# ygjwd12345/UCD

Measured on AMD Instinct MI355X. Metric: images/sec (whole node) per UCD train step, VOC 15-5 step-1, 513^2 bs=24, higher is better.
Workload: dtype bf16

## Files before the change

### include/ucd_hip.h

```cpp
#ifndef UCD_HIP_H
#define UCD_HIP_H

#include <stddef.h>
#include <stdint.h>

#ifdef __cplusplus
extern "C" {
#endif

#define UCD_VERSION 100

typedef void* ucd_stream_t;
typedef void* ucd_comm_t;

enum ucd_dtype { UCD_F32 = 0, UCD_BF16 = 1 };
enum ucd_act { UCD_ACT_IDENTITY = 0, UCD_ACT_LEAKY_RELU = 1, UCD_ACT_ELU = 2  };
#define UCD_ACT_MASK 0xff
#define UCD_NORM_ABS_GAMMA 0x100
enum ucd_pixcon_precision { UCD_PIXCON_F32 = 0, UCD_PIXCON_F16 = 1, UCD_PIXCON_F16_SPLIT = 2 };
enum ucd_error {
  UCD_OK = 0,
  UCD_EINVAL = -1,
  UCD_EALIGN = -2,
  UCD_EWORKSPACE = -3,
// ... 324 lines not shown
int ucd_abn_reduce_partials(const float* partial, int tiles, int C, float* sums, float* sums_copy, const float* weight,
                            int flags, ucd_stream_t stream);

size_t ucd_conv1x1_wgrad_workspace_bytes(int M, int N, int K);
int ucd_conv1x1_wgrad(const void* dy, int ld_dy, const void* a, int lda, int M, int N, int K,
                      const float* in_mean, const float* in_scale, const float* in_shift, int in_act, float in_slope,
                      void* dw, void* workspace, size_t workspace_bytes, ucd_stream_t stream);

int ucd_abn_sync_finalize(const float* gathered, int world, int M, int C, const float* weight, float* running_mean,
                          float* running_var, float momentum, float eps, float* buf, int flags, ucd_stream_t stream);

int ucd_stem_conv7x7(const float* x, long long sb, long long sc, long long sh, long long sw, int B, int H, int W, const void* w,
                     void* z, ucd_stream_t stream);

int ucd_stem_conv_pool(const float* x, long long sb, long long sc, long long sh, long long sw, int B, int H, int W, const void* w,
                       const float* mean, const float* scale, const float* beta, int act, float slope, void* out, ucd_stream_t stream);
int ucd_stem_pooled_size(int n);
size_t ucd_stem_pool_workspace_bytes(int C);
int ucd_stem_apply_pool(const void* z, int B, int H, int W, int C, const float* mean, const float* scale, const float* beta, int act,
                        float slope, void* out, uint8_t* idx, ucd_stream_t stream);
int ucd_stem_pool_backward(const void* z, const void* dpool, const uint8_t* idx, int B, int H, int W, int C, const float* mean,
                           const float* invstd, const float* scale, const float* beta, const float* weight, float* sums, float count,
                           int act, float slope, void* dz, void* workspace, size_t workspace_bytes, int phase, ucd_stream_t stream);

size_t ucd_conv_wgrad_workspace_bytes(int M, int N, int K, int taps);
int ucd_conv_wgrad_ex(const void* dz, int ld_dz, const void* x, int ld_x, int M, int N, int K, int taps, int H, int W, int dilation,
                      int stride, void* dw, float* dw32, int accumulate32, void* workspace, size_t workspace_bytes, int flags,
                      ucd_stream_t stream);
int ucd_conv_wgrad_defer(int mode);
int ucd_conv_wgrad_mode(void);
int ucd_conv_wgrad_flush(ucd_stream_t stream);
int ucd_conv_wgrad_drop(ucd_stream_t stream);
int ucd_conv_wgrad_drop_all(void);

enum ucd_wgrad_form {
  UCD_WGRAD_TILE = 0,
  UCD_WGRAD_STRIDED = 1,
  UCD_WGRAD_ROW3 = 2
};
#define UCD_WGRAD_FORM_NAMES {"tile", "strided", "row3"}
typedef struct ucd_conv_wgrad_plan_t {
  int form;
  int tile_n, tile_k, tiles_n, tiles_k;
  int chunks, rows_per_chunk, ksplit;
  int x_tile_rows;
  int grid, threads, lds_bytes;
// ... 60 lines not shown
```

### ucd_amd/abn.py

```python
from __future__ import annotations

import os

from . import switches as _switches

import torch
import torch.distributed as dist
import torch.nn as nn
from torch.optim.optimizer import register_optimizer_step_post_hook

from . import hip
from .comm import direct_comm


def _act_code(name):
    try:
        return hip.ACT_CODES[name]
    except KeyError:
        raise RuntimeError(f"activation {name!r} is not supported by the HIP ABN (leaky_relu, elu, identity)") from None


_param_epoch = [0]


def _after_optimizer_step(optimizer, args, kwargs):
# ... 252 lines not shown

    @staticmethod
    def forward(ctx, x):
        x, M, Cc, HW, ld = hip.rows_view(x)
        B = x.shape[0]
        out = torch.empty(B, Cc, dtype=torch.float32, device=x.device)
        hip.plane_sum(x, ld, B, HW, Cc, 1.0 / HW, out)
        ctx.shape, ctx.dtype = x.shape, x.dtype
        return out.to(x.dtype).view(B, Cc, 1, 1)

    @staticmethod
    def backward(ctx, g):
        B, Cc, H, W = ctx.shape
        return (g.to(ctx.dtype) / (H * W)).expand(B, Cc, H, W)


def global_avg_pool(x):
    return _PlaneMean.apply(x)


class _StemABNPoolFunction(torch.autograd.Function):

    @staticmethod
    def forward(ctx, z, weight, bias, running_mean, running_var, training, momentum, eps, act, slope, group, eval_consts):
        B, Cc, H, W = z.shape
        M, HW = B * H * W, H * W
        zr, _, _, _, ld = hip.rows_view(z)
        dev = z.device
        world = _group_size(group) if training else 1
        sync = training and group is not False and (world > 1 or (_FORCE_SYNC and dist.is_initialized()))
        if training:
            buf = torch.empty(((8 + 2 * world) if sync else 6) * Cc, dtype=torch.float32, device=dev)
            if sync:
                pack = buf[6 * Cc:8 * Cc]
                hip.abn_sync_stats(zr, ld, M, Cc, None, HW, buf[:2 * Cc], buf[2 * Cc:3 * Cc], pack)
                comm = direct_comm(group)
                if comm is not None:
                    gathered = buf[8 * Cc:]
                    hip._check(hip.load().ucd_comm_all_gather(comm.handle, hip.ptr(pack), hip.ptr(gathered), 2 * Cc, hip.stream()),
                               "ucd_comm_all_gather")
                else:
                    gathered = _all_gather_stats(pack, world, group)
                hip.abn_sync_finalize(gathered, world, M, Cc, weight, running_mean, running_var, momentum, eps, buf, act)
            else:
                hip.abn_stats_finalize(zr, ld, M, Cc, None, HW, buf[:2 * Cc], buf[2 * Cc:3 * Cc], weight, running_mean, running_var,
                                       momentum, eps, buf[3 * Cc:4 * Cc], buf[4 * Cc:5 * Cc], buf[5 * Cc:6 * Cc], act)
            mean, invstd, scale = buf[3 * Cc:4 * Cc], buf[4 * Cc:5 * Cc], buf[5 * Cc:6 * Cc]
        else:
            mean, invstd, scale = running_mean, eval_consts[0], eval_consts[1]
        need_bwd = any(ctx.needs_input_grad[:3])
        out, idx = hip.stem_apply_pool(z, mean, scale, bias, act, slope, need_bwd)
        if need_bwd:
            ctx.save_for_backward(z, idx, weight, bias, mean, invstd, scale)
            ctx.cfg = (training, act, slope, group, world, sync, float(M * world))
        return out

    @staticmethod
    def backward(ctx, dp):
        z, idx, weight, bias, mean, invstd, scale = ctx.saved_tensors
        training, act, slope, group, world, sync, count = ctx.cfg
        if not training:
            raise RuntimeError("ucd_amd.abn: the fused stem has no frozen-statistics backward (fix_bn keeps the separate layers)")
        Cc = z.shape[1]
        if dp.dtype != z.dtype:
            dp = dp.to(z.dtype)
        if not dp.is_contiguous(memory_format=torch.channels_last):
            dp = dp.contiguous(memory_format=torch.channels_last)
        sums = torch.empty(2 * Cc, dtype=torch.float32, device=z.device)
        dz = torch.empty_like(z) if ctx.needs_input_grad[0] else None
        if not sync:
            hip.stem_pool_backward(z, dp, idx, mean, invstd, scale, bias, weight, sums, count, act, slope, dz, 3 if dz is not None else 1)
            dbias, dweight = sums[:Cc], sums[Cc:]
        else:
            hip.stem_pool_backward(z, dp, idx, mean, invstd, scale, bias, weight, sums, count, act, slope, None, 1)
            local = sums.clone()
            dbias, dweight = local[:Cc], local[Cc:]
            comm = direct_comm(group)
            if comm is not None:
                hip._check(hip.load().ucd_comm_all_reduce_sum(comm.handle, hip.ptr(sums), 2 * Cc, hip.stream()), "ucd_comm_all_reduce_sum")
            else:
                _all_reduce_sums(sums, group)
            if dz is not None:
                hip.stem_pool_backward(z, dp, idx, mean, invstd, scale, bias, weight, sums, count, act, slope, dz, 2)
        return (dz, dweight if weight is not None else None, dbias if bias is not None else None) + (None,) * 9


def stem_norm_pool(bn, z):
    import os
    if _switches.get("UCD_STEM_FOLD", "1") == "0" or not getattr(bn, "ucd_fused_abn", False):
        return None
    Cc = z.shape[1] if z.dim() == 4 else 0
    if not (z.is_cuda and z.dim() == 4 and z.dtype == torch.bfloat16 and z.is_contiguous(memory_format=torch.channels_last)
            and z.shape[2] > 2 and z.shape[3] > 2 and Cc % 8 == 0 and 2048 % max(Cc, 1) == 0
            and bn.activation in ("leaky_relu", "identity")):
        return None
    needs_grad = torch.is_grad_enabled() and (z.requires_grad or (bn.weight is not None and bn.weight.requires_grad))
    if needs_grad and not bn.training:
        return None
    act = _act_code(bn.activation) | (hip.NORM_ABS_GAMMA if bn._abs_gamma else 0)
    if bn.training:
        bn.__dict__.pop("_eval_cache", None)
    return _StemABNPoolFunction.apply(z, bn.weight, bn.bias, bn.running_mean, bn.running_var, bn.training, bn.momentum, bn.eps, act,
                                      bn.activation_param, bn._group(), None if bn.training else bn._eval_constants())


class ABN(nn.Module):

    ucd_fused_abn = True
    _inplace_contract = False
    _sync = False
    _abs_gamma = False

    def __init__(self, num_features, eps=1e-5, momentum=0.1, affine=True, activation="leaky_relu",
                 activation_param=0.01, group=None):
        super().__init__()
        self.num_features, self.eps, self.momentum, self.affine = num_features, eps, momentum, affine
        self.activation, self.activation_param = activation, activation_param
        self.group = group
        if affine:
            self.weight = nn.Parameter(torch.ones(num_features))
            self.bias = nn.Parameter(torch.zeros(num_features))
        else:
            self.register_parameter("weight", None)
            self.register_parameter("bias", None)
        self.register_buffer("running_mean", torch.zeros(num_features))
        self.register_buffer("running_var", torch.ones(num_features))
# ... 92 lines not shown
```

### ucd_amd/backbone.py

```python
from __future__ import annotations

import sys
from collections import OrderedDict
from functools import partial

import torch
import torch.nn as nn

from . import switches as _switches
from .blocks import Conv2d, ResidualBlock, try_index

_STAGE_DILATION = {16: (1, 1, 1, 2), 8: (1, 1, 2, 4)}


class GlobalAvgPool2d(nn.Module):

    def forward(self, inputs):
        return inputs.flatten(2).mean(dim=2)


class ResNet(nn.Module):
    def __init__(self, structure, bottleneck, norm_act=nn.BatchNorm2d, classes=0,
                 output_stride=16, keep_outputs=False):
        super().__init__()
# ... 34 lines not shown
                from .abn import stem_norm_pool
                y = _stem_eval_fused(m.conv1, m.bn1, x)
                if y is not None:
                    return y
                z = _stem_conv(m.conv1, x)
                y = stem_norm_pool(m.bn1, z)
                return y if y is not None else pool(m.bn1(z))
        return m(x)

    def forward(self, x, taps=False):
        outs = [self._stem(x)]
        for name in ("mod2", "mod3", "mod4", "mod5"):
            y = getattr(self, name)(outs[-1])
            if taps and name != "mod5" and hasattr(y, "_ucd_blink"):
                del y._ucd_blink
            outs.append(y)
        if taps:
            return outs[4], tuple(outs[1:5])
        if hasattr(self, "classifier"):
            outs.append(self.classifier(outs[-1]))
        return outs if self.keep_outputs else outs[-1]


class _StemConvFunction(torch.autograd.Function):

    @staticmethod
    def forward(ctx, x, w):
        from . import hip
        ctx.save_for_backward(x, w)
        return hip.stem_conv7x7(x, w)

    @staticmethod
    def backward(ctx, dz):
        x, w = ctx.saved_tensors
        dw = None
        if ctx.needs_input_grad[1]:
            xb = x.to(torch.bfloat16).contiguous(memory_format=torch.channels_last)
            dw = torch.ops.aten.convolution_backward(dz.contiguous(memory_format=torch.channels_last), xb, w, None, [2, 2], [3, 3],
                                                     [1, 1], False, [0, 0], 1, [False, True, False])[1]
        return None, dw


def _stem_conv(conv, x):
    w = conv.working_weight() if hasattr(conv, "working_weight") else None
    if w is None and x.is_cuda and torch.is_autocast_enabled() and torch.get_autocast_dtype("cuda") == torch.bfloat16:
        w = conv.weight.to(torch.bfloat16)
    if (w is None or not x.is_cuda or x.dim() != 4 or x.dtype != torch.float32 or x.requires_grad or conv.bias is not None
            or tuple(conv.weight.shape) != (64, 3, 7, 7) or conv.stride != (2, 2) or conv.padding != (3, 3)
            or conv.dilation != (1, 1) or w.dtype != torch.bfloat16 or not w.is_contiguous(memory_format=torch.channels_last)
            or _switches.get("UCD_OWN_STEM", "1") == "0"):
        return conv(x)
    if torch.is_grad_enabled() and w.requires_grad:
        return _StemConvFunction.apply(x, w)
    from . import hip
    return hip.stem_conv7x7(x, w)


def _stem_eval_fused(conv, bn, x):
    from . import abn as _abn
    if (torch.is_grad_enabled() or bn.training or _switches.get("UCD_STEM_EVAL_FUSED", "1") == "0" or _switches.get("UCD_OWN_STEM", "1") == "0"
            or _switches.get("UCD_STEM_FOLD", "1") == "0" or not getattr(bn, "ucd_fused_abn", False)
            or bn.activation not in ("leaky_relu", "identity")):
        return None
# ... 21 lines not shown
```

### ucd_amd/csrc/stem.hip

```cpp
#include "common.h"

namespace ucd {
namespace {

typedef __hip_bfloat16 bf16;
constexpr int kThreads = 256;
constexpr int kRedBlocks = 1024;
constexpr int kApplyRows = 4;

__device__ __forceinline__ float leaky(float z, float slope) { return z > 0.f ? z : z * slope; }
__device__ __forceinline__ float bf16_round(float v) { return __bfloat162float(__float2bfloat16(v)); }

struct StemArgs {
  const bf16* z; int B, H, W, C, PH, PW;
  const float *mean, *scale, *beta, *invstd, *weight, *sums;
  float slope, inv_count;
  int abs_gamma, cg_shift;
};

__global__ __launch_bounds__(kThreads) void stem_apply_pool_kernel(StemArgs p, bf16* __restrict__ out, uint8_t* __restrict__ idx) {
  const int cgs = p.cg_shift, CG = 1 << cgs;
  const int t = blockIdx.x * kThreads + threadIdx.x;
  const int cg = t & (CG - 1), pw = t >> cgs, ph = blockIdx.y, b = blockIdx.z;
  if (pw >= p.PW) return;
// ... 419 lines not shown
    }
    __syncthreads();
    for (int i = tid; i < kFPH * kFPW * 8; i += kThreads) {
      const int cg = i & 7, pp = i >> 3, pr = pp / kFPW, pc = pp - pr * kFPW;
      const int ph = (oy0 + 1) / 2 + pr, pw = (ox0 + 1) / 2 + pc;
      if (ph >= q.PH || pw >= q.PW) continue;
      float best[8];
#pragma unroll
      for (int e = 0; e < 8; ++e) best[e] = -INFINITY;
#pragma unroll
      for (int kh = 0; kh < 3; ++kh)
#pragma unroll
        for (int kw = 0; kw < 3; ++kw) {
          Vec<bf16> v;
          v.raw = *reinterpret_cast<const uint4*>(Tl + ((2 * pr + kh) * kSTW + 2 * pc + kw) * kFTP + cg * 8);
#pragma unroll
          for (int e = 0; e < 8; ++e) best[e] = fmaxf(best[e], v.get(e));
        }
      Vec<bf16> o;
#pragma unroll
      for (int e = 0; e < 8; ++e) o.set(e, best[e]);
      o.store(q.out + (((size_t)b * q.PH + ph) * q.PW + pw) * 64 + cg * 8);
    }
  }
}

bool stem_args_ok(const void* z, int B, int H, int W, int C) {
  return z && B > 0 && B < 65536 && H > 1 && H < 65536 && W > 1 && C >= 8 && (C & (C - 1)) == 0 && C <= 2048 && aligned16(z);
}

}
}

using namespace ucd;

extern "C" {

int ucd_stem_pooled_size(int n) { return (n + 2 - 3) / 2 + 1; }

size_t ucd_stem_pool_workspace_bytes(int C) { return (size_t)kRedBlocks * 2 * C * sizeof(float); }

int ucd_stem_apply_pool(const void* z, int B, int H, int W, int C, const float* mean, const float* scale, const float* beta, int act,
                        float slope, void* out, uint8_t* idx, ucd_stream_t stream) {
  static const char* fn = "ucd_stem_apply_pool";
  UCD_REQUIRE(stem_args_ok(z, B, H, W, C) && mean && scale && out && aligned16(out) && (!idx || (reinterpret_cast<uintptr_t>(idx) & 7) == 0),
              UCD_EINVAL, "%s: dense channels-last bf16 maps with a power-of-two channel count in 8..2048 expected", fn);
// ... 54 lines not shown
  StemArgs p{};
  p.z = (const bf16*)z; p.B = B; p.H = H; p.W = W; p.C = C; p.PH = ucd_stem_pooled_size(H); p.PW = ucd_stem_pooled_size(W);
  p.mean = mean; p.scale = scale; p.beta = beta; p.invstd = invstd; p.weight = weight; p.sums = sums;
  p.slope = a == UCD_ACT_IDENTITY ? 1.f : slope; p.abs_gamma = (act & UCD_NORM_ABS_GAMMA) != 0;
  p.cg_shift = __builtin_ctz(C / 8);
  hipStream_t s = (hipStream_t)stream;
  if (phase & 1) {
    UCD_REQUIRE(workspace && workspace_bytes >= ucd_stem_pool_workspace_bytes(C), UCD_EWORKSPACE, "%s: workspace too small", fn);
    stem_pool_bwd_reduce_kernel<<<kRedBlocks, kThreads, kThreads * 16 * sizeof(float), s>>>(p, (const bf16*)dpool, idx, (float*)workspace);
    int rc = check_launch(fn);
    if (rc) return rc;
    stem_sum_partials_kernel<<<2 * C, kThreads, 0, s>>>((const float*)workspace, kRedBlocks, C, p.abs_gamma ? weight : nullptr, sums);
    rc = check_launch(fn);
    if (rc) return rc;
  }
  if (phase & 2) {
    p.inv_count = 1.f / count;
    stem_pool_bwd_apply_kernel<<<dim3(ceil_div(((W + 1) / 2) * (C / 8), kThreads), ceil_div(H, kApplyRows), B), kThreads, 0, s>>>(p, (const bf16*)dpool, idx, (bf16*)dz);
    return check_launch(fn);
  }
  return 0;
}

}
```

### ucd_amd/hip.py

```python
from __future__ import annotations

import ctypes as C
import os

import torch

_HERE = os.path.dirname(os.path.abspath(__file__))
LIB_PATH = os.path.join(_HERE, "libucd_hip.so")

F32, BF16 = 0, 1
ACT_IDENTITY, ACT_LEAKY_RELU, ACT_ELU = 0, 1, 2
ACT_CODES = {"identity": ACT_IDENTITY, "leaky_relu": ACT_LEAKY_RELU, "elu": ACT_ELU}
ACT_MASK = 0xFF
NORM_ABS_GAMMA = 0x100
PIX_TILE = 128
PIXCON_LD = 256
PIXCON_F32, PIXCON_F16, PIXCON_F16_SPLIT = 0, 1, 2
KD_UNBIASED, KD_PLAIN = 0, 1
EINVAL, EALIGN, EWORKSPACE = -1, -2, -3
EUNSUPPORTED = -4
SEG_FORMS = {1: "pk<16,8>", 2: "pk<20,4>", 3: "pk<12,12>", 4: "reg<24,16>", 5: "reg<24,24>", 6: "wide/fixed", 7: "wide/f32"}
PIXCON_PATHS = {1: "f32", 2: "f32/wide", 3: "f16/planned", 4: "f16/split"}
CONV_FORMS = ("single", "2x64", "lw/128", "lw/256", "lw/64")
WGRAD_FORMS = ("tile", "strided", "row3")
PIXCON_PRECISION = {"f32": PIXCON_F32, "fp32": PIXCON_F32, "f16": PIXCON_F16, "fp16": PIXCON_F16,
                    "f16_split": PIXCON_F16_SPLIT}


class PixconMeta(C.Structure):
    _fields_ = [("A", C.c_int32), ("Co", C.c_int32), ("min_new", C.c_int32), ("n_new", C.c_int32),
# ... 8 lines not shown

class Conv1x1Desc(C.Structure):
    _fields_ = [("a", C.c_void_p), ("lda", C.c_int), ("w", C.c_void_p), ("ldw", C.c_int), ("y", C.c_void_p), ("ldy", C.c_int),
                ("M", C.c_int), ("N", C.c_int), ("K", C.c_int),
                ("in_mean", C.c_void_p), ("in_scale", C.c_void_p), ("in_shift", C.c_void_p), ("in_act", C.c_int),
                ("in_slope", C.c_float), ("out_mode", C.c_int),
                ("out_mean", C.c_void_p), ("out_scale", C.c_void_p), ("out_shift", C.c_void_p), ("out_invstd", C.c_void_p),
                ("residual", C.c_void_p), ("ldr", C.c_int), ("out_act", C.c_int), ("out_slope", C.c_float),
                ("partial", C.c_void_p), ("accumulate", C.c_int),
                ("taps", C.c_int), ("H", C.c_int), ("W", C.c_int), ("dilation", C.c_int),
                ("side2", C.c_void_p), ("ld2", C.c_int), ("stride", C.c_int),
                ("stat_acc", C.c_void_p), ("stat_shift", C.c_void_p), ("stat_acc2", C.c_void_p), ("stat_rep", C.c_int)]


class Conv1x1Plan(C.Structure):
    _fields_ = [(n, C.c_int) for n in ("form", "tile_rows", "tile_cols", "tiles_m", "tiles_n", "grid", "threads", "lds_bytes",
                                       "param_off")]


class Conv_WgradPlan(C.Structure):
    _fields_ = [(n, C.c_int) for n in ("form", "tile_n", "tile_k", "tiles_n", "tiles_k", "chunks", "rows_per_chunk", "ksplit",
                                       "x_tile_rows", "grid", "threads", "lds_bytes", "sum_lanes", "sum_blocks")] + \
               [("workspace_bytes", C.c_size_t)]


_p, _i, _f, _z = C.c_void_p, C.c_int, C.c_float, C.c_size_t
SIGNATURES = {
    "ucd_version": (_i, []),
    "ucd_last_error": (C.c_char_p, []),
    "ucd_abn_workspace_bytes": (_z, [_i, _i]),
    "ucd_abn_stats": (_i, [_p, _i, _i, _i, _i, _p, _i, _p, _p, _p, _z, _p]),
    "ucd_abn_stats_finalize": (_i, [_p, _i, _i, _i, _i, _p, _i, _p, _p, _p, _p, _p, _f, _f, _p, _p, _p, _i, _p, _z, _p]),
    "ucd_abn_finalize": (_i, [_p, _p, _f, _i, _p, _p, _p, _f, _f, _p, _p, _p, _i, _p]),
    "ucd_abn_eval_params": (_i, [_p, _p, _f, _i, _p, _p, _i, _p]),
    "ucd_abn_apply": (_i, [_p, _i, _p, _i, _p, _i, _i, _i, _i, _p, _i, _p, _p, _p, _i, _f, _p]),
    "ucd_conv1x1_stat_replicas": (_i, [_i]),
    "ucd_fill_zero": (_i, [_p, _z, _p]),
    "ucd_abn_apply_stats": (_i, [_p, _i, _p, _i, _p, _i, _i, _i, _p, _i, _p, _f, _p, _p, _p, _p, _f, _f, _p, _p, _p, _i, _f, _p]),
    "ucd_abn_bwd_apply_raw": (_i, [_p, _i, _p, _i, _p, _i, _p, _i, _p, _i, _i, _i, _p, _p, _p, _p, _p, _p, _p, _i, _p, _f, _i, _f, _p]),
    "ucd_abn_bwd_reduce": (_i, [_p, _i, _p, _i, _p, _i, _i, _i, _i, _p, _i, _p, _p, _p, _p, _p, _i, _f, _p, _p, _z, _p]),
    "ucd_label_path": (_i, [_p, _p, _i, _i, _p, _p, _p, _p]),
    "ucd_image_path": (_i, [_p, _p, _i, _i, _i, _i, _f, _f, _f, _f, _f, _f, _p, _p, _p, _p]),
    "ucd_batch_path": (_i, [_p, _p, _p, _i, _i, _p, _f, _f, _f, _f, _f, _f, _p, _p, _p]),
    "ucd_val_image_path": (_i, [_p, _p, _i, _i, _i, _i, _i, _i, _f, _f, _f, _f, _f, _f, _p, _p, _p, _p]),
    "ucd_val_label_path": (_i, [_p, _p, _i, _i, _i, _p, _p, _p, _p]),
    "ucd_gemm_load": (_i, [C.c_char_p]),
# ... 35 lines not shown
    "ucd_attn_mse_workspace_bytes": (_z, [_i, _i]),
    "ucd_attn_mse": (_i, [_p, _i, _p, _i, _i, _i, _i, _i, _f, _p, _p, _i, _p, _z, _p]),
    "ucd_pod_plan": (_i, [_i, _i, _i, _p, _i, _i, _i, _p, _p, _p]),
    "ucd_pod_forward": (_i, [_p, _i, _p, _i, _i, _i, _i, _i, _i, _f, _p, _i, _f, _p, _p, _p, _z, _p]),
    "ucd_pod_backward": (_i, [_p, _i, _i, _i, _i, _i, _i, _f, _p, _i, _p, _p, _p, _i, _p]),
    "ucd_conv1x1_row_tiles": (_i, [_i]),
    "ucd_conv1x1_stats_partial_bytes": (_z, [_i, _i]),
    "ucd_conv1x1": (_i, [C.POINTER(Conv1x1Desc), _p]),
    "ucd_conv1x1_plan": (_i, [C.POINTER(Conv1x1Desc), C.POINTER(Conv1x1Plan)]),
    "ucd_conv1x1_stats_finalize": (_i, [_p, _i, _i, _p, _p, _p, _f, _f, _p, _p, _i, _p]),
    "ucd_conv3_tap_plan": (_i, [_i, _i, _i, _i, _i, _p, _p, _p]),
    "ucd_conv3_tap_classes": (_i, [_i]),
    "ucd_conv3_tap_plans_resident": (_i, []),
    "ucd_conv3_tap_stats": (_i, [_p, _p, _p]),
    "ucd_abn_reduce_partials": (_i, [_p, _i, _i, _p, _p, _p, _i, _p]),
    "ucd_conv1x1_wgrad_workspace_bytes": (_z, [_i, _i, _i]),
    "ucd_conv1x1_wgrad": (_i, [_p, _i, _p, _i, _i, _i, _i, _p, _p, _p, _i, _f, _p, _p, _z, _p]),
    "ucd_abn_sync_finalize": (_i, [_p, _i, _i, _i, _p, _p, _p, _f, _f, _p, _i, _p]),
    "ucd_stem_pooled_size": (_i, [_i]),
    "ucd_stem_pool_workspace_bytes": (_z, [_i]),
    "ucd_stem_apply_pool": (_i, [_p, _i, _i, _i, _i, _p, _p, _p, _i, _f, _p, _p, _p]),
    "ucd_stem_pool_backward": (_i, [_p, _p, _p, _i, _i, _i, _i, _p, _p, _p, _p, _p, _p, _f, _i, _f, _p, _p, _z, _i, _p]),
    "ucd_conv_wgrad_workspace_bytes": (_z, [_i, _i, _i, _i]),
    "ucd_stem_conv7x7": (_i, [_p, C.c_longlong, C.c_longlong, C.c_longlong, C.c_longlong, _i, _i, _i, _p, _p, _p]),
    "ucd_stem_conv_pool": (_i, [_p, C.c_longlong, C.c_longlong, C.c_longlong, C.c_longlong, _i, _i, _i, _p, _p, _p, _p, _i, _f, _p, _p]),
    "ucd_conv_wgrad_ex": (_i, [_p, _i, _p, _i, _i, _i, _i, _i, _i, _i, _i, _i, _p, _p, _i, _p, _z, _i, _p]),
    "ucd_conv_wgrad_defer": (_i, [_i]),
    "ucd_conv_wgrad_mode": (_i, []),
    "ucd_conv_wgrad_flush": (_i, [_p]),
    "ucd_conv_wgrad_drop": (_i, [_p]),
    "ucd_conv_wgrad_drop_all": (_i, []),
    "ucd_conv_wgrad_plan": (_i, [_i, _i, _i, _i, _i, _i, _i, _i, C.POINTER(Conv_WgradPlan)]),
    "ucd_transpose_bf16": (_i, [_p, _i, _i, _p, _p]),
    "ucd_conv_f32": (_i, [_p, _i, _p, _i, _p, _i, _i, _i, _i, _i, _i, _i, _i, _i, _p]),
    "ucd_conv_f32_wgrad_workspace_bytes": (_z, [_i, _i, _i, _i]),
    "ucd_conv_f32_wgrad": (_i, [_p, _i, _p, _i, _i, _i, _i, _i, _i, _i, _i, _p, _p, _z, _p]),
    "ucd_flip_weights_batched": (_i, [_p, _p, _p, _i, _p, _p]),
    "ucd_flip_weights_batched64": (_i, [_p, _p, _p, _i, _p, _p]),
    "ucd_sgd_chunk": (_i, []),
    "ucd_sgd_step": (_i, [_p, _p, _i, _p, _p]),
    "ucd_sgd_hyper_store": (_i, [_p, _p, _p]),
    "ucd_sgd_step_dev": (_i, [_p, _p, _i, _p, _p]),
    "ucd_reg_chunk": (_i, []),
    "ucd_reg_hyper_store": (_i, [_p, _p, _p]),
    "ucd_reg_step": (_i, [_p, _p, _i, _i, _p, _p, _p, _p]),
    "ucd_pixcon_prep_workspace_bytes": (_z, [_i, _i]),
# ... 582 lines not shown
    lib = load()
    B, Cc, H, W = z.shape
    PH, PW = lib.ucd_stem_pooled_size(H), lib.ucd_stem_pooled_size(W)
    out = torch.empty((B, Cc, PH, PW), dtype=z.dtype, device=z.device, memory_format=torch.channels_last)
    idx = torch.empty((B, PH, PW, Cc), dtype=torch.uint8, device=z.device) if want_idx else None
    with _timed("ucd_stem_apply_pool", (z.numel() + out.numel()) * 2 + (idx.numel() if idx is not None else 0)):
        _check(lib.ucd_stem_apply_pool(ptr(z), B, H, W, Cc, ptr(mean), ptr(scale), ptr(beta), act, float(slope), ptr(out), ptr(idx),
                                       stream()), "ucd_stem_apply_pool")
    return out, idx


def stem_pool_backward(z, dpool, idx, mean, invstd, scale, beta, weight, sums, count, act, slope, dz, phase):
    lib = load()
    B, Cc, H, W = z.shape
    nbytes = lib.ucd_stem_pool_workspace_bytes(Cc)
    ws = workspace(nbytes, z.device)
    work = (z.numel() * (2 if phase & 1 else 0) + (2 * z.numel() * 2 if phase & 2 else 0) + dpool.numel() * 3 * (1 + (phase == 3)))
    with _timed("ucd_stem_pool_backward", work):
        _check(lib.ucd_stem_pool_backward(ptr(z), ptr(dpool), ptr(idx), B, H, W, Cc, ptr(mean), ptr(invstd), ptr(scale), ptr(beta),
                                          ptr(weight), ptr(sums), float(count), act, float(slope), ptr(dz), ptr(ws), nbytes,
                                          int(phase), stream()), "ucd_stem_pool_backward")


def wgrad_defer(mode):
    return int(load().ucd_conv_wgrad_defer(int(mode) & 3))


def _wgrad_side_release(stream=None):
    from . import abn as _abn
    node = _abn._abn_node()
    if node is not None:
        node.wgrad_side_release(stream)


def wgrad_flush():
    s = stream()
    _check(load().ucd_conv_wgrad_flush(s), "ucd_conv_wgrad_flush")
    _wgrad_side_release(s)


def wgrad_drop():
    s = stream()
    rc = load().ucd_conv_wgrad_drop(s)
    if rc == 0:
        _wgrad_side_release(s)
    return rc
# ... 140 lines not shown
```

### ucd_amd/switches.py

```python
from __future__ import annotations

import os

DEFAULTS = {
    "UCD_FUSED_CONV1X1": "1",
    "UCD_BWD_LINK": "1",
    "UCD_BLOCK_LINK": "1",
    "UCD_PROJ_ALIAS": "1",
    "UCD_DGRAD_VIA_FWD": "1",
    "UCD_OWN_STRIDED": "1",
    "UCD_OWN_WGRAD": "1",
    "UCD_F32_OWN_CONV": "0",
    "UCD_OWN_HEADS": "1",
    "UCD_OWN_STEM": "1",
    "UCD_WGRAD3": "1",
    "UCD_CONV_PIPE": "auto",
    "UCD_CONV_BN64_TILES": "128",
    "UCD_CONV_LW64_TILES": "128",
    "UCD_WGRAD_DEFER": "1",
    "UCD_WGRAD_STREAM": "1",
    "UCD_CONV3_TAP_CLASSES": "1",
    "UCD_STAT_ATOMIC": "1",
    "UCD_SEG_PK": "1",
    "UCD_SEG_KD_EX": "1",
    "UCD_FUSED_LDE": "1",
    "UCD_FUSED_POD": "1",
    "UCD_VAL_DEVICE": "1",
    "UCD_STEM_EVAL_FUSED": "1",
    "UCD_STEM_FOLD": "1",
    "UCD_ABN_NODE": "1",
    "UCD_SGD": "hip",
    "UCD_STEP_GRAPH": "auto",
    "UCD_TEACHER_OVERLAP": "1",
    "UCD_DIRECT_RCCL": "1",
    "UCD_IPC_SYNC": "auto",
    "UCD_IPC_TIMEOUT_MS": "60000",
    "UCD_DDP_LATE_COPY": "1",
    "UCD_DDP_DIRECT": "auto",
    "UCD_FORCE_COLLECTIVES": "0",
}

_cache: dict = {}


def get(name: str, default: str | None = None) -> str:
    v = _cache.get(name)
    if v is None:
        if default is None:
            default = DEFAULTS.get(name, "")
        v = _cache[name] = os.environ.get(name, default)
    return v

# ... 18 lines not shown
```

Measured before the change: 845.6.

## Fuse stem pool/ABN backward with 7x7 conv weight gradient in one MFMA kernel

```diff
diff --git a/include/ucd_hip.h b/include/ucd_hip.h
--- a/include/ucd_hip.h
+++ b/include/ucd_hip.h
@@ -370,6 +370,17 @@
 int ucd_stem_pool_backward(const void* z, const void* dpool, const uint8_t* idx, int B, int H, int W, int C, const float* mean,
                            const float* invstd, const float* scale, const float* beta, const float* weight, float* sums, float count,
                            int act, float slope, void* dz, void* workspace, size_t workspace_bytes, int phase, ucd_stream_t stream);
+
+typedef struct ucd_stem_wgrad_plan_t {
+  int OH, OW, tiles_y, tiles_x, tiles, min_tiles, workgroups, lds_bytes, supported, qualifies;
+  size_t workspace_bytes;
+} ucd_stem_wgrad_plan_t;
+int ucd_stem_wgrad_plan(int B, int H, int W, int workgroups, ucd_stem_wgrad_plan_t* plan);
+int ucd_stem_pool_backward_wgrad(const void* z, const void* dpool, const uint8_t* idx, int B, int OH, int OW, const float* mean,
+                                 const float* invstd, const float* scale, const float* beta, const float* weight, float* sums,
+                                 float count, int act, float slope, const void* dz, const float* x, long long sb, long long sc,
+                                 long long sh, long long sw, int H, int W, void* dw, void* workspace, size_t workspace_bytes,
+                                 int phase, int workgroups, ucd_stream_t stream);
 
 size_t ucd_conv_wgrad_workspace_bytes(int M, int N, int K, int taps);
 int ucd_conv_wgrad_ex(const void* dz, int ld_dz, const void* x, int ld_x, int M, int N, int K, int taps, int H, int W, int dilation,
diff --git a/ucd_amd/abn.py b/ucd_amd/abn.py
--- a/ucd_amd/abn.py
+++ b/ucd_amd/abn.py
@@ -1,6 +1,7 @@
 from __future__ import annotations
 
 import os
+import weakref
 
 from . import switches as _switches
 
@@ -299,7 +300,8 @@
 class _StemABNPoolFunction(torch.autograd.Function):
 
     @staticmethod
-    def forward(ctx, z, weight, bias, running_mean, running_var, training, momentum, eps, act, slope, group, eval_consts):
+    def forward(ctx, z, weight, bias, running_mean, running_var, training, momentum, eps, act, slope, group, eval_consts,
+                link, zref):
         B, Cc, H, W = z.shape
         M, HW = B * H * W, H * W
         zr, _, _, _, ld = hip.rows_view(z)
@@ -330,6 +332,7 @@
         if need_bwd:
             ctx.save_for_backward(z, idx, weight, bias, mean, invstd, scale)
             ctx.cfg = (training, act, slope, group, world, sync, float(M * world))
+            ctx.link, ctx.zref = link, zref
         return out
 
     @staticmethod
@@ -344,6 +347,26 @@
         if not dp.is_contiguous(memory_format=torch.channels_last):
             dp = dp.contiguous(memory_format=torch.channels_last)
         sums = torch.empty(2 * Cc, dtype=torch.float32, device=z.device)
+        link = ctx.link
+        if link is not None and ctx.needs_input_grad[0]:
+            zt = ctx.zref() if ctx.zref is not None else None
+            if zt is None or not (zt.retains_grad or zt._backward_hooks):
+                args = dict(z=z, dpool=dp, idx=idx, mean=mean, invstd=invstd, scale=scale, beta=bias, weight=weight, sums=sums,
+                            count=count, act=act, slope=slope)
+                if not sync:
+                    link.dw = hip.stem_pool_backward_wgrad(link.x, phase=3, **args)
+                    dbias, dweight = sums[:Cc], sums[Cc:]
+                else:
+                    hip.stem_pool_backward(z, dp, idx, mean, invstd, scale, bias, weight, sums, count, act, slope, None, 1)
+                    local = sums.clone()
+                    dbias, dweight = local[:Cc], local[Cc:]
+                    comm = direct_comm(group)
+                    if comm is not None:
+                        hip._check(hip.load().ucd_comm_all_reduce_sum(comm.handle, hip.ptr(sums), 2 * Cc, hip.stream()), "ucd_comm_all_reduce_sum")
+                    else:
+                        _all_reduce_sums(sums, group)
+                    link.dw = hip.stem_pool_backward_wgrad(link.x, phase=2, **args)
+                return (None, dweight if weight is not None else None, dbias if bias is not None else None) + (None,) * 11
         dz = torch.empty_like(z) if ctx.needs_input_grad[0] else None
         if not sync:
             hip.stem_pool_backward(z, dp, idx, mean, invstd, scale, bias, weight, sums, count, act, slope, dz, 3 if dz is not None else 1)
@@ -359,7 +382,7 @@
                 _all_reduce_sums(sums, group)
             if dz is not None:
                 hip.stem_pool_backward(z, dp, idx, mean, invstd, scale, bias, weight, sums, count, act, slope, dz, 2)
-        return (dz, dweight if weight is not None else None, dbias if bias is not None else None) + (None,) * 9
+        return (dz, dweight if weight is not None else None, dbias if bias is not None else None) + (None,) * 11
 
 
 def stem_norm_pool(bn, z):
@@ -377,8 +400,10 @@
     act = _act_code(bn.activation) | (hip.NORM_ABS_GAMMA if bn._abs_gamma else 0)
     if bn.training:
         bn.__dict__.pop("_eval_cache", None)
+    link = z.__dict__.pop("_ucd_stem_link", None)
     return _StemABNPoolFunction.apply(z, bn.weight, bn.bias, bn.running_mean, bn.running_var, bn.training, bn.momentum, bn.eps, act,
-                                      bn.activation_param, bn._group(), None if bn.training else bn._eval_constants())
+                                      bn.activation_param, bn._group(), None if bn.training else bn._eval_constants(),
+                                      link, weakref.ref(z) if link is not None else None)
 
 
 class ABN(nn.Module):
diff --git a/ucd_amd/backbone.py b/ucd_amd/backbone.py
--- a/ucd_amd/backbone.py
+++ b/ucd_amd/backbone.py
@@ -80,23 +80,43 @@
         return outs if self.keep_outputs else outs[-1]
 
 
+class StemLink:
+    __slots__ = ("x", "dw")
+
+    def __init__(self, x):
+        self.x, self.dw = x, None
+
+
 class _StemConvFunction(torch.autograd.Function):
 
     @staticmethod
     def forward(ctx, x, w):
         from . import hip
         ctx.save_for_backward(x, w)
-        return hip.stem_conv7x7(x, w)
+        z = hip.stem_conv7x7(x, w)
+        ctx.link = None
+        if ctx.needs_input_grad[1] and hip.stem_wgrad_mode(x):
+            ctx.link = z._ucd_stem_link = StemLink(x)
+            ctx.set_materialize_grads(False)
+        return z
 
     @staticmethod
     def backward(ctx, dz):
         x, w = ctx.saved_tensors
         dw = None
+        if dz is None:
+            if ctx.link is not None:
+                dw, ctx.link.dw = ctx.link.dw, None
+            return None, dw
         if ctx.needs_input_grad[1]:
-            xb = x.to(torch.bfloat16).contiguous(memory_format=torch.channels_last)
-            dw = torch.ops.aten.convolution_backward(dz.contiguous(memory_format=torch.channels_last), xb, w, None, [2, 2], [3, 3],
-                                                     [1, 1], False, [0, 0], 1, [False, True, False])[1]
+            dw = _stem_wgrad_library(x, w, dz)
         return None, dw
+
+
+def _stem_wgrad_library(x, w, dz):
+    xb = x.to(torch.bfloat16).contiguous(memory_format=torch.channels_last)
+    return torch.ops.aten.convolution_backward(dz.contiguous(memory_format=torch.channels_last), xb, w, None, [2, 2], [3, 3],
+                                               [1, 1], False, [0, 0], 1, [False, True, False])[1]
 
 
 def _stem_conv(conv, x):
diff --git a/ucd_amd/csrc/stem.hip b/ucd_amd/csrc/stem.hip
--- a/ucd_amd/csrc/stem.hip
+++ b/ucd_amd/csrc/stem.hip
@@ -465,6 +465,195 @@
       for (int e = 0; e < 8; ++e) o.set(e, best[e]);
       o.store(q.out + (((size_t)b * q.PH + ph) * q.PW + pw) * 64 + cg * 8);
     }
+  }
+}
+
+constexpr int kGP = 264;
+constexpr int kWgradSlab = 64 * kSK;
+constexpr int kWgradMaxWgs = 512;
+constexpr int kWgradMinTiles = 256;
+constexpr int kWgradLds = (kSIR * kSIP + 64 * kGP) * 2 + 7 * 64 * 4;
+constexpr int kSumOuts = 16, kSumParts = kThreads / kSumOuts;
+
+struct StemWgradArgs {
+  StemArgs s;
+  const bf16* dpool; const uint8_t* idx;
+  const bf16* dz;
+  const float* x; long long sb, sc, sh, sw;
+  float* slabs;
+  int IH, IW, tiles_y, tiles_x, ntiles;
+};
+
+template <bool FUSED>
+__global__ __launch_bounds__(kThreads, 2) void stem_pool_bwd_wgrad_kernel(StemWgradArgs q) {
+  typedef float f32x16 __attribute__((ext_vector_type(16)));
+  typedef __bf16 bf16x8 __attribute__((ext_vector_type(8)));
+  __shared__ __attribute__((aligned(16))) unsigned short In[kSIR * kSIP];
+  __shared__ __attribute__((aligned(16))) unsigned short Gt[64 * kGP];
+  const StemArgs& p = q.s;
+  const int tid = threadIdx.x, lane = tid & 63, wave = tid >> 6;
+  const int col = lane & 31, h = lane >> 5;
+  const int cg = tid & 7, cp = (tid >> 3) & 15, qr = tid >> 7;
+  __shared__ float Pc[7 * 64];
+  if (FUSED && tid < 64) {
+    const int ch = tid;
+    const float sc = p.scale[ch], is = p.invstd[ch];
+    float k1 = p.sums[p.C + ch] * p.inv_count, gw;
+    if (p.abs_gamma) {
+      if (p.weight && p.weight[ch] < 0.f) k1 = -k1;
+      gw = sc;
+    } else {
+      gw = (p.weight ? p.weight[ch] : 1.f) * is;
+    }
+    Pc[ch] = p.mean[ch]; Pc[64 + ch] = sc; Pc[128 + ch] = p.beta ? p.beta[ch] : 0.f; Pc[192 + ch] = is;
+    Pc[256 + ch] = p.sums[ch] * p.inv_count; Pc[320 + ch] = k1; Pc[384 + ch] = gw;
+  }
+  const int nb = wave & 1, kb0 = (wave >> 1) * 3;
+  int pbase[3];
+#pragma unroll
+  for (int j = 0; j < 3; ++j) {
+    const int kc = (kb0 + j) * 32 + col, ky = kc / 24 > 6 ? 6 : kc / 24;
+    pbase[j] = ky * kSIP + (kc % 24) + 48 * h;
+  }
+  f32x16 acc[3];
+#pragma unroll
+  for (int j = 0; j < 3; ++j)
+#pragma unroll
+    for (int r = 0; r < 16; ++r) acc[j][r] = 0.f;
+  const int fe = tid < kSIP ? tid : kSIP - 1, fpx = fe / 3, fc = fe - fpx * 3;
+  float pre[kSIR];
+  unsigned premask = 0;
+  auto fetch = [&](int tile) {
+    unsigned okm = 0;
+    const int b = tile / (q.tiles_y * q.tiles_x), rem = tile - b * q.tiles_y * q.tiles_x;
+    const int oy0 = (rem / q.tiles_x) * kSTH, ox0 = (rem % q.tiles_x) * kSTW;
+    const int ix = 2 * ox0 - 3 + fpx;
+    const bool colok = fpx < 2 * kSTW + 5 && (unsigned)ix < (unsigned)q.IW;
+    const float* src = q.x + b * q.sb + fc * q.sc + (colok ? ix : 0) * q.sw;
+#pragma unroll
+    for (int r = 0; r < kSIR; ++r) {
+      const int iy = 2 * oy0 - 3 + r;
+      const bool ok = colok && (unsigned)iy < (unsigned)q.IH;
+      pre[r] = src[(ok ? iy : 0) * q.sh];
+      okm |= ok ? (1u << r) : 0u;
+    }
+    premask = okm;
+  };
+  if ((int)blockIdx.x < q.ntiles) fetch(blockIdx.x);
+  for (int tile = blockIdx.x; tile < q.ntiles; tile += gridDim.x) {
+    const int b = tile / (q.tiles_y * q.tiles_x), rem = tile - b * q.tiles_y * q.tiles_x;
+    const int oy0 = (rem / q.tiles_x) * kSTH, ox0 = (rem % q.tiles_x) * kSTW;
+    const int y0 = oy0 + kApplyRows * qr, i = ox0 / 2 + cp, x0 = 2 * i, phb = y0 / 2;
+    Vec<bf16> g[3][2], v[kApplyRows][2];
+    uint2 w[3][2];
+    bool gv[3][2];
+    if (FUSED) {
+#pragma unroll
+      for (int a = 0; a < 3; ++a)
+#pragma unroll
+        for (int c = 0; c < 2; ++c) {
+          gv[a][c] = phb + a < p.PH && i + c < p.PW;
+          const size_t off = (((size_t)b * p.PH + min(phb + a, p.PH - 1)) * p.PW + min(i + c, p.PW - 1)) * p.C + cg * 8;
+          w[a][c] = *reinterpret_cast<const uint2*>(q.idx + off);
+          g[a][c].load(q.dpool + off);
+        }
+    }
+    const bf16* vsrc = FUSED ? p.z : q.dz;
+#pragma unroll
+    for (int r = 0; r < kApplyRows; ++r)
+#pragma unroll
+      for (int cx = 0; cx < 2; ++cx)
+        v[r][cx].load(vsrc + (((size_t)b * p.H + min(y0 + r, p.H - 1)) * p.W + min(x0 + cx, p.W - 1)) * p.C + cg * 8);
+    __syncthreads();
+    if (tid < kSIP) {
+#pragma unroll
+      for (int r = 0; r < kSIR; ++r) {
+        const bf16 t = __float2bfloat16((premask >> r) & 1u ? pre[r] : 0.f);
+        In[r * kSIP + tid] = *reinterpret_cast<const unsigned short*>(&t);
+      }
+    }
+#pragma unroll
+    for (int e = 0; e < 8; ++e) {
+      const int ch = cg * 8 + e;
+      float mu = 0.f, sc = 0.f, sh = 0.f, is = 0.f, k0 = 0.f, k1 = 0.f, gw = 0.f;
+      if (FUSED) { mu = Pc[ch]; sc = Pc[64 + ch]; sh = Pc[128 + ch]; is = Pc[192 + ch]; k0 = Pc[256 + ch]; k1 = Pc[320 + ch]; gw = Pc[384 + ch]; }
+      unsigned* dst = reinterpret_cast<unsigned*>(&Gt[ch * kGP + kApplyRows * qr * kSTW + 2 * cp]);
+#pragma unroll
+      for (int r = 0; r < kApplyRows; ++r) {
+        unsigned bits[2];
+#pragma unroll
+        for (int cx = 0; cx < 2; ++cx) {
+          const bool inside = y0 + r < p.H && x0 + cx < p.W;
+          if (FUSED) {
+            float dy = 0.f;
+#pragma unroll
+            for (int ya = 0; ya < 2; ++ya) {
+              if (ya == 1 && !(r & 1)) continue;
+              const int a = (r >> 1) + ya, kh = (r & 1) ? (ya ? 0 : 2) : 1;
+#pragma unroll
+              for (int xa = 0; xa < 2; ++xa) {
+                if (xa == 1 && !cx) continue;
+                const int kw = cx ? (xa ? 0 : 2) : 1;
+                const unsigned pos = gv[a][xa] ? (unsigned)(kh * 3 + kw) : 0xffu;
+                const unsigned id = ((e < 4 ? w[a][xa].x : w[a][xa].y) >> (8 * (e & 3))) & 0xffu;
+                dy += id == pos ? g[a][xa].get(e) : 0.f;
+              }
+            }
+            const float xc = v[r][cx].get(e) - mu;
+            const float dza = dy * (xc * sc + sh > 0.f ? 1.f : p.slope);
+            const bf16 t = __float2bfloat16((dza - k0 - (xc * is) * k1) * gw);
+            bits[cx] = *reinterpret_cast<const unsigned short*>(&t);
+          } else {
+            bits[cx] = ((&v[r][cx].raw.x)[e >> 1] >> (16 * (e & 1))) & 0xffffu;
+          }
+          if (!inside) bits[cx] = 0u;
+        }
+        dst[r * (kSTW / 2)] = bits[0] | (bits[1] << 16);
+      }
+    }
+    __syncthreads();
+    if (tile + (int)gridDim.x < q.ntiles) fetch(tile + gridDim.x);
+#pragma unroll
+    for (int s = 0; s < kSTH * kSTW / 16; ++s) {
+      const bf16x8 gf = *reinterpret_cast<const bf16x8*>(&Gt[(nb * 32 + col) * kGP + 16 * s + 8 * h]);
+      bf16x8 pf[3];
+#pragma unroll
+      for (int j = 0; j < 3; ++j) {
+        const unsigned short* src = &In[pbase[j] + (s >> 1) * 2 * kSIP + (s & 1) * 96];
+        union { unsigned u[4]; bf16x8 v; } f;
+#pragma unroll
+        for (int e = 0; e < 4; ++e) f.u[e] = (unsigned)src[12 * e] | ((unsigned)src[12 * e + 6] << 16);
+        pf[j] = f.v;
+      }
+#pragma unroll
+      for (int j = 0; j < 3; ++j) acc[j] = __builtin_amdgcn_mfma_f32_32x32x16_bf16(gf, pf[j], acc[j], 0, 0, 0);
+    }
+  }
+  float* slab = q.slabs + (size_t)blockIdx.x * kWgradSlab;
+#pragma unroll
+  for (int j = 0; j < 3; ++j) {
+    const int kc = (kb0 + j) * 32 + col;
+    if (kc >= kSK) continue;
+#pragma unroll
+    for (int r = 0; r < 16; ++r) slab[(nb * 32 + (r & 3) + 8 * (r >> 2) + 4 * h) * kSK + kc] = acc[j][r];
+  }
+}
+
+__global__ __launch_bounds__(kThreads) void stem_wgrad_sum_kernel(const float* __restrict__ slabs, int nslabs, bf16* __restrict__ dw) {
+  __shared__ float red[kThreads];
+  const int o = threadIdx.x % kSumOuts, part = threadIdx.x / kSumOuts, i = blockIdx.x * kSumOuts + o;
+  float s = 0.f;
+  if (i < 64 * 147) {
+    const int n = i / 147, r = i - n * 147, ky = r / 21, j = r - ky * 21;
+    const float* src = slabs + n * kSK + ky * 24 + j;
+#pragma unroll 8
+    for (int k = part; k < nslabs; k += kSumParts) s += src[(size_t)k * kWgradSlab];
+  }
+  red[threadIdx.x] = s;
+  __syncthreads();
+  if (part == 0 && i < 64 * 147) {
+    for (int k = 1; k < kSumParts; ++k) s += red[k * kSumOuts + o];
+    dw[i] = __float2bfloat16(s);
   }
 }
 
@@ -565,4 +754,70 @@
   return 0;
 }
 
-}
+int ucd_stem_wgrad_plan(int B, int H, int W, int workgroups, ucd_stem_wgrad_plan_t* plan) {
+  static const char* fn = "ucd_stem_wgrad_plan";
+  UCD_REQUIRE(plan, UCD_EINVAL, "%s: NULL plan", fn);
+  *plan = ucd_stem_wgrad_plan_t{};
+  UCD_REQUIRE(B > 0 && H > 0 && W > 0 && workgroups >= 0 && workgroups <= 65535, UCD_EINVAL, "%s: bad arguments", fn);
+  plan->OH = (H + 6 - 7) / 2 + 1; plan->OW = (W + 6 - 7) / 2 + 1;
+  plan->tiles_y = ceil_div(plan->OH, kSTH); plan->tiles_x = ceil_div(plan->OW, kSTW);
+  const long long tiles = (long long)B * plan->tiles_y * plan->tiles_x;
+  plan->supported = B < 65536 && plan->OH > 1 && plan->OH < 65536 && plan->OW > 1 && tiles < (1ll << 30);
+  if (!plan->supported) return 0;
+  plan->tiles = (int)tiles;
+  plan->min_tiles = kWgradMinTiles;
+  plan->qualifies = plan->tiles >= kWgradMinTiles;
+  plan->workgroups = workgroups > 0 ? workgroups : (plan->tiles < kWgradMaxWgs ? plan->tiles : kWgradMaxWgs);
+  plan->lds_bytes = kWgradLds;
+  const size_t slabs = (size_t)plan->workgroups * kWgradSlab * sizeof(float), red = ucd_stem_pool_workspace_bytes(64);
+  plan->workspace_bytes = slabs > red ? slabs : red;
+  return 0;
+}
+
+int ucd_stem_pool_backward_wgrad(const void* z, const void* dpool, const uint8_t* idx, int B, int OH, int OW, const float* mean,
+                                 const float* invstd, const float* scale, const float* beta, const float* weight, float* sums,
+                                 float count, int act, float slope, const void* dz, const float* x, long long sb, long long sc,
+                                 long long sh, long long sw, int H, int W, void* dw, void* workspace, size_t workspace_bytes,
+                                 int phase, int workgroups, ucd_stream_t stream) {
+  static const char* fn = "ucd_stem_pool_backward_wgrad";
+  ucd_stem_wgrad_plan_t pl;
+  int rc = ucd_stem_wgrad_plan(B, H, W, workgroups, &pl);
+  if (rc) return rc;
+  UCD_REQUIRE(pl.supported && pl.OH == OH && pl.OW == OW, UCD_EINVAL, "%s: an image [%d, 3, %d, %d] with its [%d, 64, %d, %d] map expected",
+              fn, B, H, W, B, pl.OH, pl.OW);
+  UCD_REQUIRE(x && dw && (reinterpret_cast<uintptr_t>(dw) & 1) == 0 && (phase == 0 || phase == 2 || phase == 3), UCD_EINVAL,
+              "%s: bad arguments", fn);
+  UCD_REQUIRE(workspace && aligned16(workspace) && workspace_bytes >= pl.workspace_bytes, UCD_EWORKSPACE, "%s: workspace too small", fn);
+  StemWgradArgs q{};
+  StemArgs& p = q.s;
+  p.B = B; p.H = OH; p.W = OW; p.C = 64; p.PH = ucd_stem_pooled_size(OH); p.PW = ucd_stem_pooled_size(OW);
+  q.x = x; q.sb = sb; q.sc = sc; q.sh = sh; q.sw = sw; q.IH = H; q.IW = W; q.slabs = (float*)workspace;
+  q.tiles_y = pl.tiles_y; q.tiles_x = pl.tiles_x; q.ntiles = pl.tiles;
+  hipStream_t s = (hipStream_t)stream;
+  if (phase == 0) {
+    UCD_REQUIRE(dz && aligned16(dz), UCD_EINVAL, "%s: dense channels-last bf16 dz expected", fn);
+    q.dz = (const bf16*)dz;
+    stem_pool_bwd_wgrad_kernel<false><<<pl.workgroups, kThreads, 0, s>>>(q);
+  } else {
+    UCD_REQUIRE(stem_args_ok(z, B, OH, OW, 64) && dpool && idx && mean && invstd && scale && sums && aligned16(dpool) && count > 0.f &&
+                (reinterpret_cast<uintptr_t>(idx) & 7) == 0, UCD_EINVAL, "%s: bad arguments", fn);
+    const int a = act & UCD_ACT_MASK;
+    UCD_REQUIRE(a != UCD_ACT_ELU, UCD_EUNSUPPORTED, "%s: leaky_relu / identity only", fn);
+    if (phase == 3) {
+      rc = ucd_stem_pool_backward(z, dpool, idx, B, OH, OW, 64, mean, invstd, scale, beta, weight, sums, count, act, slope, nullptr,
+                                  workspace, workspace_bytes, 1, stream);
+      if (rc) return rc;
+    }
+    p.z = (const bf16*)z; p.mean = mean; p.scale = scale; p.beta = beta; p.invstd = invstd; p.weight = weight; p.sums = sums;
+    p.slope = a == UCD_ACT_IDENTITY ? 1.f : slope; p.abs_gamma = (act & UCD_NORM_ABS_GAMMA) != 0;
+    p.cg_shift = 3; p.inv_count = 1.f / count;
+    q.dpool = (const bf16*)dpool; q.idx = idx;
+    stem_pool_bwd_wgrad_kernel<true><<<pl.workgroups, kThreads, 0, s>>>(q);
+  }
+  rc = check_launch(fn);
+  if (rc) return rc;
+  stem_wgrad_sum_kernel<<<ceil_div(64 * 147, kSumOuts), kThreads, 0, s>>>((const float*)workspace, pl.workgroups, (bf16*)dw);
+  return check_launch(fn);
+}
+
+}
diff --git a/ucd_amd/hip.py b/ucd_amd/hip.py
--- a/ucd_amd/hip.py
+++ b/ucd_amd/hip.py
@@ -5,7 +5,9 @@
 
 import torch
 
-_HERE = os.path.dirname(os.path.abspath(__file__))
+from . import switches as _switches
+
+_HERE =os.path.dirname(os.path.abspath(__file__))
 LIB_PATH = os.path.join(_HERE, "libucd_hip.so")
 
 F32, BF16 = 0, 1
@@ -60,6 +62,11 @@
     _fields_ = [(n, C.c_int) for n in ("form", "tile_n", "tile_k", "tiles_n", "tiles_k", "chunks", "rows_per_chunk", "ksplit",
                                        "x_tile_rows", "grid", "threads", "lds_bytes", "sum_lanes", "sum_blocks")] + \
                [("workspace_bytes", C.c_size_t)]
+
+
+class StemWgradPlan(C.Structure):
+    _fields_ = [(n, C.c_int) for n in ("OH", "OW", "tiles_y", "tiles_x", "tiles", "min_tiles", "workgroups", "lds_bytes",
+                                       "supported", "qualifies")] + [("workspace_bytes", C.c_size_t)]
 
 
 _p, _i, _f, _z = C.c_void_p, C.c_int, C.c_float, C.c_size_t
@@ -141,6 +148,9 @@
     "ucd_stem_apply_pool": (_i, [_p, _i, _i, _i, _i, _p, _p, _p, _i, _f, _p, _p, _p]),
     "ucd_stem_pool_backward": (_i, [_p, _p, _p, _i, _i, _i, _i, _p, _p, _p, _p, _p, _p, _f, _i, _f, _p, _p, _z, _i, _p]),
     "ucd_conv_wgrad_workspace_bytes": (_z, [_i, _i, _i, _i]),
+    "ucd_stem_wgrad_plan": (_i, [_i, _i, _i, _i, C.POINTER(StemWgradPlan)]),
+    "ucd_stem_pool_backward_wgrad": (_i, [_p, _p, _p, _i, _i, _i, _p, _p, _p, _p, _p, _p, _f, _i, _f, _p, _p, C.c_longlong, C.c_longlong,
+                                          C.c_longlong, C.c_longlong, _i, _i, _p, _p, _z, _i, _i, _p]),
     "ucd_stem_conv7x7": (_i, [_p, C.c_longlong, C.c_longlong, C.c_longlong, C.c_longlong, _i, _i, _i, _p, _p, _p]),
     "ucd_stem_conv_pool": (_i, [_p, C.c_longlong, C.c_longlong, C.c_longlong, C.c_longlong, _i, _i, _i, _p, _p, _p, _p, _i, _f, _p, _p]),
     "ucd_conv_wgrad_ex": (_i, [_p, _i, _p, _i, _i, _i, _i, _i, _i, _i, _i, _i, _p, _p, _i, _p, _z, _i, _p]),
@@ -769,6 +779,47 @@
                                           int(phase), stream()), "ucd_stem_pool_backward")
 
 
+def stem_wgrad_plan(B, H, W, workgroups=0):
+    p = StemWgradPlan()
+    _check(load().ucd_stem_wgrad_plan(int(B), int(H), int(W), int(workgroups), C.byref(p)), "ucd_stem_wgrad_plan")
+    return {n: getattr(p, n) for n, _ in StemWgradPlan._fields_}
+
+
+def stem_wgrad_mode(x):
+    mode = _switches.get("UCD_STEM_WGRAD", "1")
+    if mode == "0" or x.dim() != 4 or x.shape[1] != 3 or x.dtype != torch.float32:
+        return False
+    plan = stem_wgrad_plan(x.shape[0], x.shape[2], x.shape[3])
+    return bool(plan["supported"] if mode == "2" else plan["qualifies"])
+
+
+def stem_pool_backward_wgrad(x, dz=None, z=None, dpool=None, idx=None, mean=None, invstd=None, scale=None, beta=None, weight=None,
+                             sums=None, count=1.0, act=0, slope=0.0, phase=0, workgroups=0):
+    lib = load()
+    B, _, H, W = x.shape
+    plan = stem_wgrad_plan(B, H, W, workgroups)
+    if not plan["supported"]:
+        raise RuntimeError(f"ucd_stem_pool_backward_wgrad: image {tuple(x.shape)} is not a shape the stem backward takes")
+    OH, OW = plan["OH"], plan["OW"]
+    ref = dz if phase == 0 else z
+    if tuple(ref.shape) != (B, 64, OH, OW) or ref.dtype != torch.bfloat16 or not ref.is_contiguous(memory_format=torch.channels_last):
+        raise RuntimeError("ucd_stem_pool_backward_wgrad: a dense channels-last bf16 map [B, 64, OH, OW] expected")
+    dw = torch.empty((64, 3, 7, 7), dtype=torch.bfloat16, device=x.device, memory_format=torch.channels_last)
+    nbytes = plan["workspace_bytes"]
+    ws = workspace(nbytes, x.device)
+    sb, sc, sh, sw = x.stride()
+    if phase == 0:
+        work = dz.numel() * 2 + x.numel() * 4
+    else:
+        work = z.numel() * 2 * (2 if phase == 3 else 1) + x.numel() * 4 + dpool.numel() * 3 * (2 if phase == 3 else 1)
+    with _timed("ucd_stem_pool_backward", work):
+        _check(lib.ucd_stem_pool_backward_wgrad(ptr(z), ptr(dpool), ptr(idx), B, OH, OW, ptr(mean), ptr(invstd), ptr(scale), ptr(beta),
+                                                ptr(weight), ptr(sums), float(count), int(act), float(slope), ptr(dz), ptr(x),
+                                                sb, sc, sh, sw, H, W, ptr(dw), ptr(ws), nbytes, int(phase), int(workgroups),
+                                                stream()), "ucd_stem_pool_backward_wgrad")
+    return dw
+
+
 def wgrad_defer(mode):
     return int(load().ucd_conv_wgrad_defer(int(mode) & 3))
 
diff --git a/ucd_amd/switches.py b/ucd_amd/switches.py
--- a/ucd_amd/switches.py
+++ b/ucd_amd/switches.py
@@ -28,6 +28,7 @@
     "UCD_VAL_DEVICE": "1",
     "UCD_STEM_EVAL_FUSED": "1",
     "UCD_STEM_FOLD": "1",
+    "UCD_STEM_WGRAD": "1",
     "UCD_ABN_NODE": "1",
     "UCD_SGD": "hip",
     "UCD_STEP_GRAPH": "auto",
```

Result: no change. 850.3, median of 6 (+0.6%).
